# minh86/ModelCrowdNav

Measured on AMD Instinct MI355X. Metric: env-steps/sec (whole node), 5-human CrowdSim x batched envs, higher is better.
Workload: dtype f64

## Files before the change

modelcrowdnav_amd/csrc/env_rollout_wg4.hip:

```cpp
#include "env_rollout_common.hpp"

namespace mcn {

template <int NT>
struct Wg4 {
    static_assert(NT == 5, "the four-wavefront form is built for 5 humans only");
    static constexpr int EW = 8;
    static constexpr int NQ = EW * NT;
};

template <int CTRL>
__device__ __forceinline__ int dpp_i(int v) { return __builtin_amdgcn_mov_dpp(v, CTRL, 0xf, 0xf, true); }
template <int CTRL>
__device__ __forceinline__ double dpp_d(double v)
{
    const long long b = __builtin_bit_cast(long long, v);
    const int lo = dpp_i<CTRL>((int)b), hi = dpp_i<CTRL>((int)(b >> 32));
    return __builtin_bit_cast(double, ((long long)hi << 32) | (unsigned int)lo);
}
constexpr int DPP_QUAD_XOR1 = 0xB1, DPP_QUAD_XOR2 = 0x4E, DPP_ROW_HALF_MIRROR = 0x141;

template <int NT, int VIS, bool UNI>
__device__ __forceinline__ void rollout_wg4(const StepParams &p, const int T)
{
    static_assert(VIS == 0, "the four-wavefront form is built for an invisible robot only");
    constexpr int EW = Wg4<NT>::EW, NQ = Wg4<NT>::NQ;
    __shared__ float4 s_pack[NQ];
    __shared__ float2 s_res[2 * NQ], s_inv[NQ];
    __shared__ double2 s_hpos[NQ];
    __shared__ double s_hrad[NQ];
    __shared__ float4 s_lines[3 * 64];
    STAMP(0);
    STAMP_WHERE();
#ifdef MCN_DIAG
    if (p.debug_noop) return;
#endif
    const int tid = threadIdx.x;
    const int role = __builtin_amdgcn_readfirstlane(tid >> 6);
    const unsigned chunk_ = xcd_chunk();
    const mcn_env_cfg &c = p.cfg;
    const mcn_rollout &ro = p.roll;

    if (role < 3) {
        const int lane = tid & 63, k = tid & 3, q = tid >> 2;
        const bool pop = q < NQ;
        const int ge = q / NT, h = q - ge * NT;
        const bool active = pop && (long)chunk_ * EW + ge < p.E;
        const int hi = pop ? q : 0;
        const bool cand_h = k < NT - 1;
        const int j = cand_h ? k + (k >= h ? 1 : 0) : h;
        const int ci = pop ? ge * NT + j : 0;
        const bool publish = pop && k == 0;
        const float inv_th = in_vgpr(1.0f / c.orca_time_horizon), inv_ts = in_vgpr(1.0f / (float)c.time_step);
        constexpr int RES_BUF = NQ * (int)sizeof(float2);
        const int hi_b = hi * (int)sizeof(float2), ci_b = ci * (int)sizeof(float2);
        int rd_h = hi_b + RES_BUF, rd_c = ci_b + RES_BUF;
        const char *res_bytes = reinterpret_cast<const char *>(s_res);
        const QuadTable lines = {s_lines + role * 64};
        __syncthreads();
        STAMP(1);

        for (int t = 0; t < T; ++t) {
            float4 P = s_pack[hi];
            float2 cp = *reinterpret_cast<const float2 *>(s_pack + ci);
            float2 v = *reinterpret_cast<const float2 *>(res_bytes + rd_h), cv = *reinterpret_cast<const float2 *>(res_bytes + rd_c);
            float2 fm = s_inv[hi];
            float orad = s_inv[ci].x;
            asm volatile("" : "+v"(P.x), "+v"(P.y), "+v"(P.z), "+v"(P.w), "+v"(cp.x), "+v"(cp.y), "+v"(v.x), "+v"(v.y),
                              "+v"(cv.x), "+v"(cv.y), "+v"(fm.x), "+v"(fm.y), "+v"(orad));
            float rx, ry;
            quad_orca_core(c, lane, k, cand_h && active, make_float4(P.x, P.y, v.x, v.y), make_float4(P.z, P.w, fm.x, fm.y),
                           make_float4(cp.x, cp.y, cv.x, cv.y), orad, inv_th, inv_ts, rx, ry, lines);
            if (publish) s_res[(t & 1) * NQ + hi] = make_float2(rx, ry);
            rd_h = in_vgpr(hi_b + (t & 1) * RES_BUF); rd_c = in_vgpr(ci_b + (t & 1) * RES_BUF);
            if (t < 20) STAMP(40 + t);
            __syncthreads();
            __syncthreads();
            if (t < 37) STAMP(2 + t);
        }
    } else {
        static_assert(EW * 8 == 64, "eight lanes per env fill the wavefront");
        const double dt = in_vgpr(c.time_step);
        const bool do_reset = p.has_roll && ro.pool_hpos != nullptr;
        const int l = tid & 63;
        const int g = l >> 3, h = l & 7;
        const bool pop = h < NT;
        const int hs = g * NT + (pop ? h : 0);
        const long e = (long)chunk_ * EW + g;
        const bool active = pop && e < p.E;
        const long eb = e < p.E ? e : 0;
        const long a = eb * NT + (pop ? h : 0);
        const bool lead = active && h == 0;
        constexpr bool unicycle = UNI;
        const bool has_state = p.has_roll && ro.state != nullptr;
        const bool track = c.track_human_times && p.st.human_times != nullptr;

        double2 pos = reinterpret_cast<const double2 *>(p.st.hpos)[a];
        double2 vel = reinterpret_cast<const double2 *>(p.st.hvel)[a];
        double2 goal = reinterpret_cast<const double2 *>(p.st.hgoal)[a];
        double rad = p.st.hrad[a];
        double vpref = p.st.hvpref[a];
        double htime = p.st.human_times ? p.st.human_times[a] : 0.0;
        double hax = 0, hay = 0;
        double2 rpos = reinterpret_cast<const double2 *>(p.st.rpos)[eb];
        double2 rvel = reinterpret_cast<const double2 *>(p.st.rvel)[eb];
        double2 rgoal = reinterpret_cast<const double2 *>(p.st.rgoal)[eb];
        const double rrad = p.st.rrad[eb];
        double gtime = p.st.gtime[eb];
        double rtheta = p.st.rtheta ? p.st.rtheta[eb] : 0.0;
        mcn_roll_rec rs = {0, 0, 0, 0, 0, 0};
        if (has_state) rs = ro.state[eb];
        const double2 *act_ptr = reinterpret_cast<const double2 *>(p.actions) + eb;
        const long act_stride = in_vgpr((long)p.E);
        const double *disc_table = in_vgpr(ro.disc_table);
        const int disc_last = in_vgpr(ro.disc_len - 1);
        const bool has_theta = p.st.rtheta != nullptr;
        double2 act_next = *act_ptr;
        double o_rew = 0, o_dmin = 0;
        int o_dn = 0, o_inf = 0, o_hh = 0;
        const double k_timeout_at = in_vgpr(c.time_limit - 1);
        const double k_collision = in_vgpr(c.collision_penalty), k_success = in_vgpr(c.success_reward);
        const double k_discomfort = in_vgpr(c.discomfort_dist), k_factor = in_vgpr(c.discomfort_penalty_factor);
        const int k_stride = ro.case_stride, k_pool = ro.pool_size;
        const bool count_hh = c.count_hh != 0;
        {
            float4 A, B;
            quad_orca_operands(c, pos, vel, goal, rad, vpref, A, B);
            if (pop) {
                s_pack[hs] = make_float4(A.x, A.y, B.x, B.y); s_res[NQ + hs] = make_float2(A.z, A.w);
                s_inv[hs] = make_float2(B.z, B.w);
                s_hpos[hs] = pos; s_hrad[hs] = rad;
            }
        }
        __syncthreads();
        STAMP(1);

        for (int t = 0; t < T; ++t) {
            const double2 act = act_next;
            act_ptr += act_stride;
            if (t + 1 < T) act_next = *act_ptr;
            double ep_disc = 0;
            if (has_state) ep_disc = disc_table[rs.ep_steps < disc_last ? rs.ep_steps : disc_last];

            double2 eff = act;
            if (unicycle) {
                eff.x = act.x * cos(act.y + rtheta);
                eff.y = act.x * sin(act.y + rtheta);
            }
            double cd;
            {
                const double px = pos.x - rpos.x, py = pos.y - rpos.y;
                const double vx = vel.x - eff.x, vy = vel.y - eff.y;
                cd = p2s_origin(px, py, px + vx * dt, py + vy * dt) - rad - rrad;
            }
            cd = pop ? cd : INFINITY;
            int hh = 0;
            {
                static_assert(NT / 2 == 2, "two pairs per lane");
                double s2[2], ra[2], rb[2];
                bool near_any = false;
                const bool counted = active & count_hh;
#pragma unroll
                for (int d = 1; d <= NT / 2; ++d) {
                    const int jj = h + d >= NT ? h + d - NT : h + d;
                    const int pi = g * NT + (pop ? jj : 0);
                    const double2 ppos = s_hpos[pi];
                    const double prad = s_hrad[pi];
                    ra[d - 1] = jj > h ? rad : prad; rb[d - 1] = jj > h ? prad : rad;
                    const double dx = pos.x - ppos.x, dy = pos.y - ppos.y;
                    s2[d - 1] = dx * dx + dy * dy;
                    const double reach = ra[d - 1] + rb[d - 1] + 1e-6;
                    near_any |= counted & (s2[d - 1] < reach * reach);
                }
                if (__any(near_any)) {
                    DIAG_COUNT(2);
#pragma unroll
                    for (int d = 0; d < NT / 2; ++d)
                        hh += (counted & ((sqrt(s2[d]) - ra[d] - rb[d]) < 0)) ? 1 : 0;
                }
            }
            double dmin = cd;
            int hh_sum = hh;
            dmin = fmin(dmin, dpp_d<DPP_QUAD_XOR1>(dmin));       hh_sum += dpp_i<DPP_QUAD_XOR1>(hh_sum);
            dmin = fmin(dmin, dpp_d<DPP_QUAD_XOR2>(dmin));       hh_sum += dpp_i<DPP_QUAD_XOR2>(hh_sum);
            dmin = fmin(dmin, dpp_d<DPP_ROW_HALF_MIRROR>(dmin)); hh_sum += dpp_i<DPP_ROW_HALF_MIRROR>(hh_sum);

            double endx, endy, new_theta = rtheta, nrvx, nrvy;
            if (unicycle) {
                const double th = rtheta + act.y;
                endx = rpos.x + cos(th) * act.x * dt;
                endy = rpos.y + sin(th) * act.x * dt;
                new_theta = pymod(rtheta + act.y, 2 * M_PI);
                nrvx = act.x * cos(new_theta); nrvy = act.x * sin(new_theta);
            } else {
                endx = rpos.x + act.x * dt; endy = rpos.y + act.y * dt;
                nrvx = act.x; nrvy = act.y;
            }
            bool reaching = false;
            {
                const double gx = endx - rgoal.x, gy = endy - rgoal.y, near = rrad + 1e-6;
                if (__any(gx * gx + gy * gy < near * near)) DIAG_COUNT(3);
                if (__any(gx * gx + gy * gy < near * near)) reaching = norm2(gx, gy) < rrad;
            }
            double rew; int inf, dn;
            if (gtime >= k_timeout_at)          { rew = 0; dn = 1; inf = MCN_INFO_TIMEOUT; }
            else if (dmin < 0)                  { rew = k_collision; dn = 1; inf = MCN_INFO_COLLISION; }
            else if (reaching)                  { rew = k_success; dn = 1; inf = MCN_INFO_REACHGOAL; }
            else if (dmin < k_discomfort)       { rew = (dmin - k_discomfort) * k_factor * dt; dn = 0; inf = MCN_INFO_DANGER; }
            else                                { rew = 0; dn = 0; inf = MCN_INFO_NOTHING; }
            o_rew = rew; o_dmin = dmin; o_dn = dn; o_inf = inf; o_hh = hh_sum;
            const double t_new = gtime + dt;

            const int case_g = rs.next_case;
            if (has_state) {
                bool danger = inf == MCN_INFO_DANGER;
                if (danger) {
                    const KernargPtr kp = kernarg_here();
                    const int lim = kp->roll.danger_episodes, sf = kp->roll.danger_short_from;
                    danger = lim <= 0 || rs.fin_count < lim - ((sf > 0 && e >= sf - 1) ? 1 : 0);
                }
                rs.danger_count += danger ? 1 : 0;
                rs.danger_dist_sum = danger ? rs.danger_dist_sum + dmin : rs.danger_dist_sum;
                const double ret = rs.ep_return + ep_disc * rew;
                if (lead && dn) {
                    const int kf = rs.fin_count;
                    const KernargPtr kp = kernarg_here();
                    const int fin_slots = kp->roll.fin_slots;
                    double *fin_return = kp->roll.fin_return, *fin_time = kp->roll.fin_time;
                    uint8_t *fin_info = kp->roll.fin_info;
                    const bool keep = (fin_slots == 1) || (kf < fin_slots);
                    const long rec = (long)(fin_slots == 1 ? 0 : kf) * kp->E + e;
                    if (keep && fin_return) fin_return[rec] = ret;
                    if (keep && fin_time)   fin_time[rec] = (inf == MCN_INFO_TIMEOUT) ? kp->cfg.time_limit : t_new;
                    if (keep && fin_info)   fin_info[rec] = (uint8_t)inf;
                }
                rs.fin_count += dn;
                rs.ep_return = dn ? 0.0 : ret;
                rs.ep_steps = dn ? 0 : rs.ep_steps + 1;
                if (do_reset) {
                    int nc = rs.next_case + k_stride;
                    nc = nc >= k_pool ? nc - k_pool : nc;
                    rs.next_case = dn ? nc : rs.next_case;
                }
            }

            if (do_reset && dn) {
                const KernargPtr kp = kernarg_here();
                const double k_theta0 = kp->roll.robot_theta0;
                rpos = make_double2(kp->roll.robot_start[0], kp->roll.robot_start[1]);
                rgoal = make_double2(kp->roll.robot_goal[0], kp->roll.robot_goal[1]);
                rvel = make_double2(0, 0);
                if (has_theta) rtheta = k_theta0;
                gtime = 0;
            } else {
                rpos = make_double2(endx, endy);
                rvel = make_double2(nrvx, nrvy);
                if (unicycle) rtheta = new_theta;
                gtime = t_new;
            }

            const bool restart = do_reset && dn;
            float4 n_pack = make_float4(0, 0, 0, 0);
            float2 n_fvel = make_float2(0, 0), n_inv = make_float2(0, 0);
            if (restart) {
                DIAG_COUNT(1);
                if (active) {
                    const long pa = (long)case_g * NT + h;
                    const KernargPtr kp = kernarg_here();
                    const double2 *pool_hvel = reinterpret_cast<const double2 *>(kp->roll.pool_hvel);
                    vel = make_double2(0, 0);
                    if (pool_hvel) vel = pool_hvel[pa];
                    pos = reinterpret_cast<const double2 *>(kp->roll.pool_hpos)[pa];
                    goal = reinterpret_cast<const double2 *>(kp->roll.pool_hgoal)[pa];
                    rad = kp->roll.pool_hrad[pa];
                    vpref = kp->roll.pool_hvpref[pa];
                }
                htime = 0;
                float4 A, B;
                quad_orca_operands(c, pos, vel, goal, rad, vpref, A, B);
                n_pack = make_float4(in_vgpr(A.x), in_vgpr(A.y), in_vgpr(B.x), in_vgpr(B.y));
                n_fvel = make_float2(in_vgpr(A.z), in_vgpr(A.w));
                n_inv = make_float2(in_vgpr(B.z), in_vgpr(B.w));
            }
            const bool any_restart = __any(restart);

            if (t < 20) STAMP(40 + t);
            __syncthreads();
            float2 *vel_io = s_res + (t & 1) * NQ;
            {
                const float2 r = vel_io[hs];
                hax = (double)r.x; hay = (double)r.y;
            }
            if (!restart) {
                pos = make_double2(pos.x + hax * dt, pos.y + hay * dt);
                if (pop) s_pack[hs] = quad_orca_position_pack(pos, goal);
            }
            if (any_restart) {
                if (pop && restart) { s_pack[hs] = n_pack; vel_io[hs] = n_fvel; s_inv[hs] = n_inv; }
            }
            __syncthreads();
            if (t < 37) STAMP(2 + t);

            if (pop) s_hpos[hs] = pos;
            if (!restart) {
                vel = make_double2(hax, hay);
                if (track && htime == 0 && norm2(pos.x - goal.x, pos.y - goal.y) < rad) htime = t_new;
            }
            if (any_restart) {
                if (pop && restart) s_hrad[hs] = rad;
            }
        }

        long a2 = a, e2 = e;
        asm volatile("" : "+v"(a2), "+v"(e2));
        const KernargPtr kp = kernarg_here();
        if (active) {
            reinterpret_cast<double2 *>(kp->st.hpos)[a2] = pos;
            reinterpret_cast<double2 *>(kp->st.hvel)[a2] = vel;
            if (do_reset) {
                reinterpret_cast<double2 *>(kp->st.hgoal)[a2] = goal;
                kp->st.hrad[a2] = rad;
                kp->st.hvpref[a2] = vpref;
            }
            double *human_times = kp->st.human_times, *human_act = kp->out.human_act;
            if (human_times) human_times[a2] = htime;
            if (human_act) reinterpret_cast<double2 *>(human_act)[a2] = make_double2(hax, hay);
        }
        if (lead) {
            reinterpret_cast<double2 *>(kp->st.rpos)[e2] = rpos;
            reinterpret_cast<double2 *>(kp->st.rvel)[e2] = rvel;
            if (do_reset) reinterpret_cast<double2 *>(kp->st.rgoal)[e2] = rgoal;
            double *rth = kp->st.rtheta;
            if (rth) rth[e2] = rtheta;
            kp->st.gtime[e2] = gtime;
            store_step_rec(kp->out.rec + e2, o_rew, o_dmin, o_dn, o_inf, o_hh);
            if (has_state) kp->roll.state[e2] = rs;
        }
    }
    STAMP(39);
}

template <int NT, int VIS, bool UNI>
__global__ __launch_bounds__(256, 2) void env_rollout_wg4_kernel(const StepParams p, const int T)
{
    rollout_wg4<NT, VIS, UNI>(p, T);
}

void launch_env_rollout_wg4(const StepParams &p, int T, hipStream_t stream)
{
    constexpr int NT = 5, EW = Wg4<NT>::EW;
    const dim3 grid((p.E + EW - 1) / EW), block(256);
    if (p.cfg.robot_kinematics == MCN_KIN_UNICYCLE)
        hipLaunchKernelGGL((env_rollout_wg4_kernel<NT, 0, true>), grid, block, 0, stream, p, T);
    else
        hipLaunchKernelGGL((env_rollout_wg4_kernel<NT, 0, false>), grid, block, 0, stream, p, T);
}

#ifdef MCN_DIAG
int read_counts_wg4(void *dst, size_t bytes, int reset) { return read_counts_here(dst, bytes, reset); }
int read_stamps_wg4(void *dst, size_t bytes) { return read_stamps_here(dst, bytes); }
#endif

}
```

Baseline: 2.011 billion.

## Keep ORCA velocities in registers and reload shared state only after restarts

The ORCA wavefronts now carry their own and neighbour velocities, radius and speed terms in registers across steps. They re-read s_res and s_inv from shared memory only when the dynamics wavefront raises a flag saying some environment restarted. The double-buffered result array becomes a single buffer. An extra conditional barrier is added on restart steps so both sides stay matched. This removes per-step LDS reads, but it adds a flag broadcast and makes barrier matching depend on a uniform restart flag, which is fragile.

```diff
diff --git a/modelcrowdnav_amd/csrc/env_rollout_wg4.hip b/modelcrowdnav_amd/csrc/env_rollout_wg4.hip
--- a/modelcrowdnav_amd/csrc/env_rollout_wg4.hip
+++ b/modelcrowdnav_amd/csrc/env_rollout_wg4.hip
@@ -26,7 +26,8 @@
     static_assert(VIS == 0, "the four-wavefront form is built for an invisible robot only");
     constexpr int EW = Wg4<NT>::EW, NQ = Wg4<NT>::NQ;
     __shared__ float4 s_pack[NQ];
-    __shared__ float2 s_res[2 * NQ], s_inv[NQ];
+    __shared__ float2 s_res[NQ], s_inv[NQ];
+    __shared__ int s_flag[2 * NQ];
     __shared__ double2 s_hpos[NQ];
     __shared__ double s_hrad[NQ];
     __shared__ float4 s_lines[3 * 64];
@@ -52,32 +53,38 @@
         const int ci = pop ? ge * NT + j : 0;
         const bool publish = pop && k == 0;
         const float inv_th = in_vgpr(1.0f / c.orca_time_horizon), inv_ts = in_vgpr(1.0f / (float)c.time_step);
-        constexpr int RES_BUF = NQ * (int)sizeof(float2);
-        const int hi_b = hi * (int)sizeof(float2), ci_b = ci * (int)sizeof(float2);
-        int rd_h = hi_b + RES_BUF, rd_c = ci_b + RES_BUF;
-        const char *res_bytes = reinterpret_cast<const char *>(s_res);
-        const QuadTable lines = {s_lines + role * 64};
+        float4 *const tab = s_lines + role * 64;
+        float vx = 0, vy = 0, cvx = 0, cvy = 0, frad = 0, ms = 0, orad = 0;
+        bool slow = true;
         __syncthreads();
         STAMP(1);
 
         for (int t = 0; t < T; ++t) {
             float4 P = s_pack[hi];
             float2 cp = *reinterpret_cast<const float2 *>(s_pack + ci);
-            float2 v = *reinterpret_cast<const float2 *>(res_bytes + rd_h), cv = *reinterpret_cast<const float2 *>(res_bytes + rd_c);
-            float2 fm = s_inv[hi];
-            float orad = s_inv[ci].x;
-            asm volatile("" : "+v"(P.x), "+v"(P.y), "+v"(P.z), "+v"(P.w), "+v"(cp.x), "+v"(cp.y), "+v"(v.x), "+v"(v.y),
-                              "+v"(cv.x), "+v"(cv.y), "+v"(fm.x), "+v"(fm.y), "+v"(orad));
+            if (slow) {
+                float2 v = s_res[hi], cv = s_res[ci];
+                float2 fm = s_inv[hi];
+                float od = s_inv[ci].x;
+                asm volatile("" : "+v"(v.x), "+v"(v.y), "+v"(cv.x), "+v"(cv.y), "+v"(fm.x), "+v"(fm.y), "+v"(od));
+                __syncthreads();
+                vx = v.x; vy = v.y; cvx = cv.x; cvy = cv.y; frad = fm.x; ms = fm.y; orad = od;
+            }
             float rx, ry;
-            quad_orca_core(c, lane, k, cand_h && active, make_float4(P.x, P.y, v.x, v.y), make_float4(P.z, P.w, fm.x, fm.y),
-                           make_float4(cp.x, cp.y, cv.x, cv.y), orad, inv_th, inv_ts, rx, ry, lines);
-            if (publish) s_res[(t & 1) * NQ + hi] = make_float2(rx, ry);
-            rd_h = in_vgpr(hi_b + (t & 1) * RES_BUF); rd_c = in_vgpr(ci_b + (t & 1) * RES_BUF);
+            quad_orca_core(c, lane, k, cand_h && active, make_float4(P.x, P.y, vx, vy), make_float4(P.z, P.w, frad, ms),
+                           make_float4(cp.x, cp.y, cvx, cvy), orad, inv_th, inv_ts, rx, ry, QuadTable{tab});
+            if (publish) s_res[hi] = make_float2(rx, ry);
             if (t < 20) STAMP(40 + t);
             __syncthreads();
+            int flag = s_flag[0];
+            float2 cv = s_res[ci];
+            asm volatile("" : "+v"(flag), "+v"(cv.x), "+v"(cv.y));
+            slow = __builtin_amdgcn_readfirstlane(flag) != 0;
+            vx = rx; vy = ry; cvx = cv.x; cvy = cv.y;
             __syncthreads();
             if (t < 37) STAMP(2 + t);
         }
+        if (slow) __syncthreads();
     } else {
         static_assert(EW * 8 == 64, "eight lanes per env fill the wavefront");
         const double dt = in_vgpr(c.time_step);
@@ -127,11 +134,12 @@
             float4 A, B;
             quad_orca_operands(c, pos, vel, goal, rad, vpref, A, B);
             if (pop) {
-                s_pack[hs] = make_float4(A.x, A.y, B.x, B.y); s_res[NQ + hs] = make_float2(A.z, A.w);
+                s_pack[hs] = make_float4(A.x, A.y, B.x, B.y); s_res[hs] = make_float2(A.z, A.w);
                 s_inv[hs] = make_float2(B.z, B.w);
                 s_hpos[hs] = pos; s_hrad[hs] = rad;
             }
         }
+        __syncthreads();
         __syncthreads();
         STAMP(1);
 
@@ -210,6 +218,9 @@
             else                                { rew = 0; dn = 0; inf = MCN_INFO_NOTHING; }
             o_rew = rew; o_dmin = dmin; o_dn = dn; o_inf = inf; o_hh = hh_sum;
             const double t_new = gtime + dt;
+            const bool restart = do_reset && dn;
+            const bool any_restart = __any(restart);
+            s_flag[0] = any_restart ? 1 : 0;
 
             const int case_g = rs.next_case;
             if (has_state) {
@@ -259,7 +270,6 @@
                 gtime = t_new;
             }
 
-            const bool restart = do_reset && dn;
             float4 n_pack = make_float4(0, 0, 0, 0);
             float2 n_fvel = make_float2(0, 0), n_inv = make_float2(0, 0);
             if (restart) {
@@ -282,11 +292,10 @@
                 n_fvel = make_float2(in_vgpr(A.z), in_vgpr(A.w));
                 n_inv = make_float2(in_vgpr(B.z), in_vgpr(B.w));
             }
-            const bool any_restart = __any(restart);
 
             if (t < 20) STAMP(40 + t);
             __syncthreads();
-            float2 *vel_io = s_res + (t & 1) * NQ;
+            float2 *vel_io = s_res;
             {
                 const float2 r = vel_io[hs];
                 hax = (double)r.x; hay = (double)r.y;
@@ -299,6 +308,7 @@
                 if (pop && restart) { s_pack[hs] = n_pack; vel_io[hs] = n_fvel; s_inv[hs] = n_inv; }
             }
             __syncthreads();
+            if (any_restart) __syncthreads();
             if (t < 37) STAMP(2 + t);
 
             if (pop) s_hpos[hs] = pos;
```

Result: faster. 2.039 billion (median of 6 runs) (+1.4%).
